# lightec-xyz/bls-verify-gadget

Measured on AMD Instinct MI355X. Metric: BLS-verify witness instances/sec (full pairing circuit), higher is better.
Workload: dtype u32 (381-bit Montgomery integers mod the BLS12-381 prime as 12 x 32-bit limbs in memory, products on 14 x 28-bit limbs with 64-bit columns; SHA-256 words)

## Files before the change

__graft_entry__.py:

```python
import importlib
import os
import subprocess
import sys

ROOT = os.path.dirname(os.path.abspath(__file__))
if ROOT not in sys.path:
    sys.path.insert(0, ROOT)


def build():
    pkg = importlib.import_module("bls-verify-gadget_amd")
    pkg.build(force=False)
    subprocess.check_call(["make", "-s", "-C", os.path.join(ROOT, "oracle")])
    subprocess.check_call(["make", "-s", "-C", os.path.join(ROOT, "tests", "hostsim")])
    subprocess.check_call(["make", "-s", "-C", os.path.join(ROOT, "tests", "vgroups")])
    subprocess.check_call(["make", "-s", "-j3", "-C", os.path.join(ROOT, "tests", "devfield")])
    subprocess.check_call(["make", "-s", "-j3", "-C", os.path.join(ROOT, "tests", "devcurve")])
    subprocess.check_call(["make", "-s", "-C", os.path.join(ROOT, "tests", "devteam")])
    subprocess.check_call(["make", "-s", "-C", os.path.join(ROOT, "tests", "devstream")])
    subprocess.check_call(["make", "-s", "-C", os.path.join(ROOT, "tests", "msg_input")])
    subprocess.check_call(["make", "-s", "-C", os.path.join(ROOT, "tests", "agg_inputs")])
    subprocess.check_call(["make", "-s", "-C", os.path.join(ROOT, "tests", "c_caller")])
    subprocess.check_call(["make", "-s", "-C", os.path.join(ROOT, "tests", "cpp_caller")])
    pkg.lib()
    for s in pkg.EXPORTED_SYMBOLS:
        getattr(pkg.lib(), s)


def smoke():
    import numpy as np
    import torch

    from tests import oracle_lib, synth

    pkg = importlib.import_module("bls-verify-gadget_amd")
    o = oracle_lib.load()
    n = 4
    pk, msg, sig, expect = synth.make_batch(o, n, seed=0x5EED)
    dev = torch.device("cuda:0")
    g = pkg.BlsSignatureVerifyGadget(n, 32, device=dev)
    res = g.verify(pkg.ParametersVar(), pkg.PublicKeyVar.new_witness(torch.from_numpy(pk.view(np.int64)).to(dev)),
                   torch.from_numpy(msg).to(dev), pkg.SignatureVar.new_witness(torch.from_numpy(sig.view(np.int64)).to(dev)))
    torch.cuda.synchronize()
    got = res.cpu().numpy().astype(bool)
    w = g.witness.cpu().numpy().view(np.uint64)
    for i in range(n):
        nw, _, r, ow = o.witness(pk[i], msg[i].tobytes(), sig[i])
# ... 10 lines not shown
```

bls-verify-gadget_amd/csrc/engine.hip:

```cpp
#include <cstdio>
#include <cstdlib>
#include <deque>
#include <map>
#include <vector>
#include "kcommon.hpp"
#include "agg_input.hpp"

using namespace blsw;

namespace {

inline int hip_ok(hipError_t e, const char* what) {
    if (e != hipSuccess) {
        fprintf(stderr, "[blsw] %s: %s\n", what, hipGetErrorString(e));
        return BLSW_ERR_HIP;
    }
    return BLSW_OK;
}

struct DeviceGuard {
    int prev = -1;
    bool switched = false;
    explicit DeviceGuard(int dev) {
        if (dev < 0) return;
// ... 85 lines not shown
    for (int k = 0; k < BLSW_MAX_BUFFERS; k++) {
        GroupBuf& b = e->buf[k];
        if (b.h_desc) hipHostFree(b.h_desc);
        if (b.d_desc) hipFree(b.d_desc);
        for (int i = 0; i < 2; i++)
            if (b.st[i]) hipStreamDestroy(b.st[i]);
        hipEvent_t single[] = {b.ev_start, b.ev_aux, b.ev_sha, b.ev_chains, b.ev_done, b.ev_side};
        for (hipEvent_t ev : single)
            if (ev) hipEventDestroy(ev);
        for (hipEvent_t ev : b.ev_cof)
            if (ev) hipEventDestroy(ev);
        hipEvent_t* arrays[] = {b.ev_in, b.ev_x, b.ev_step};
        for (hipEvent_t* arr : arrays) {
            if (!arr) continue;
            for (uint32_t s = 0; s < e->max_steps; s++)
                if (arr[s]) hipEventDestroy(arr[s]);
            delete[] arr;
        }
    }
    if (e->sha) hipStreamDestroy(e->sha);
    if (e->expand) hipStreamDestroy(e->expand);
    if (e->place) hipStreamDestroy(e->place);
    if (e->lat) hipStreamDestroy(e->lat);
    if (e->ev_exp) {
        for (int i = 0; i < 2 * BLSW_MAX_TIMED; i++)
            if (e->ev_exp[i]) hipEventDestroy(e->ev_exp[i]);
        delete[] e->ev_exp;
    }
    for (int i = 0; i < BLSW_MAX_CONSUMED; i++)
        if (e->consumed_ev[i]) hipEventDestroy(e->consumed_ev[i]);
    delete e;
}

static void launch_place(blsw_engine* e, hipStream_t st, const Fp* staging, const Fp* pair, uint32_t split_row, uint64_t first, uint64_t* out, uint64_t out_stride) {
    const blsw_layout_t& R = e->LR;
    const uint32_t rows = R.n_witness - R.sha_bits;
    const unsigned chunks = (rows * 3 + 256 * BLSW_PLACE_ITERS - 1) / (256 * BLSW_PLACE_ITERS);
    dim3 grid2(8 * ((chunks + 7) / 8) * (unsigned)e->n);
    const MovedSegment mv = moved_segment(R, e->modes);
    hipLaunchKernelGGL(k_place_field, grid2, dim3(256), 0, st, staging, pair, first, R.off_expand, R.sha_bits, rows, split_row, out + (uint64_t)e->head * 6, out_stride,
                       (uint32_t)e->n, mv.lo, mv.len, mv.at);
}
static void launch_place_multi(blsw_engine* e, hipStream_t st, const Workspace& ws, const Fp* pair_tiles, uint64_t first_pair, const Fp* inst_tiles, uint64_t first_inst,
                               uint32_t inst_tile_w, const Fp* rows, uint64_t* out, uint64_t out_stride) {
    const blsw_layout_t& L = e->L;
    const blsw_layout_t& S = e->LS;
    const uint32_t K = L.n_pairs, n = (uint32_t)e->n;
    PlaceRuns pr = {};
    pr.n_runs = 6;
    const uint32_t src[7] = {S.off_msg, S.off_pk_alloc, S.off_pk_not_zero, S.off_map0, S.off_prep_h, S.off_prep_pk, ws.rows_p};
    const uint32_t dst[6] = {L.off_msg, L.off_pk_alloc, L.off_pk_not_zero, L.off_map0, L.off_prep_h, L.off_prep_pk};
    const uint32_t str[6] = {L.stride_msg, L.stride_pk_alloc, L.stride_pk_not_zero, L.stride_hash, L.stride_prep_h, L.stride_prep_pk};
    for (int r = 0; r < 7; r++) pr.src_row[r] = src[r];
    for (int r = 0; r < 6; r++) pr.dst_off[r] = dst[r], pr.dst_stride[r] = str[r];
    auto blocks = [](uint32_t rows_, uint32_t n_y) {
        const unsigned chunks = (rows_ * 3 + 256 * BLSW_PLACE_ITERS - 1) / (256 * BLSW_PLACE_ITERS);
        return dim3(8 * ((chunks + 7) / 8) * n_y);
    };
    hipLaunchKernelGGL(k_place_runs, blocks(ws.rows_p, n * K), dim3(256), 0, st, pair_tiles, first_pair, ws.rows_p, pr, out, out_stride, n * K, K, 64u);
    PlaceRuns pi = {};
    pi.n_runs = 2;
    pi.src_row[0] = S.off_sig_alloc;
    pi.src_row[1] = S.off_prep_sig;
    pi.src_row[2] = ws.rows_i;
    pi.dst_off[0] = L.off_sig_alloc;
    pi.dst_off[1] = L.off_prep_sig;
    hipLaunchKernelGGL(k_place_runs, blocks(ws.rows_i, n), dim3(256), 0, st, inst_tiles, first_inst, ws.rows_i, pi, out, out_stride, n, 1u, inst_tile_w);
    const unsigned chunks = (ws.pair_rows * 3 + 256 * BLSW_PLACE_ITERS - 1) / (256 * BLSW_PLACE_ITERS);
    hipLaunchKernelGGL(k_place_rows, dim3(chunks, n), dim3(256), 0, st, rows, ws.pair_rows, L.off_miller, out, out_stride);
}
static void launch_canonical(blsw_engine* e, hipStream_t st, uint64_t* out, uint64_t out_stride) {
    const blsw_layout_t& R = e->LR;
    const uint32_t K = R.n_pairs, rows = R.n_witness - K * R.sha_bits;
    hipLaunchKernelGGL(k_canonical_rows, dim3((rows + 255) / 256, (unsigned)e->n), dim3(256), 0, st, out + (uint64_t)e->head * 6, out_stride, R.off_expand, R.sha_bits, rows, K,
// ... 29 lines not shown
        e->consumed_live[c] = false;
    }
}
static void materialise(blsw_engine* e, int k, uint32_t s) {
    GroupBuf& b = e->buf[k];
    const StepDesc& d = b.h_desc[s];
    const Workspace& ws = b.ws;
    const uint32_t Kc = e->L.n_pairs;
    const CompactForm cf = compact_form(e->n, ws, Kc);
    hipStreamWaitEvent(e->expand, b.ev_sha, 0);
    if (d.compact) {
        wait_released(e, e->expand, d.compact);
        hipMemcpyAsync(d.compact, ws.bits + (uint64_t)s * (e->n * Kc / 64) * bits_tile_words(ws.sha_words), cf.bits_bytes, hipMemcpyDeviceToDevice, e->expand);
    }
    if (d.out) {
        wait_released(e, e->expand, d.out);
        const bool timed = e->n_timed < BLSW_MAX_TIMED;
        if (timed) hipEventRecord(e->ev_exp[2 * e->n_timed], e->expand);
        const uint32_t K = e->L.n_pairs;
        ExpandArgs xa = {ws.bits, ws.sha_words, (uint64_t)s * e->n * K, e->L.sha_bits, e->L.off_expand, d.out, d.out_stride, K, K > 1 ? e->L.stride_hash : 0u, 0, (int)e->opt.output_form};
        if (b.lat_group && e->opt.consumer_mode) hipStreamWaitEvent(e->expand, b.ev_cof[2 * BLSW_COFV_NSEG + 3], 0);
        engine_expand(e, e->expand, xa, (unsigned)(e->n * K));
        if (timed) {
            hipEventRecord(e->ev_exp[2 * e->n_timed + 1], e->expand);
            e->n_timed++;
        }
        if (e->head) launch_keys_broadcast(d.ks_table, e->head, d.out, d.out_stride, e->n, 0, e->expand);
    }
    hipEventRecord(b.ev_x[s], e->expand);
    hipStreamWaitEvent(e->place, b.ev_chains, 0);
    hipStreamWaitEvent(e->place, b.ev_x[s], 0);
    if (d.compact) {
        char* dst = reinterpret_cast<char*>(d.compact);
        hipMemcpyAsync(dst + cf.off_staging, ws.staging + (uint64_t)s * (e->n * Kc / 64) * ws.rows_p * 64, cf.staging_bytes, hipMemcpyDeviceToDevice, e->place);
        if (cf.inst_bytes) {
            const uint64_t lane0 = (uint64_t)s * e->n;
            const Fp* src = ws.staging_inst + (lane0 >> 6) * (uint64_t)ws.rows_i * 64 + (lane0 & 63);
            if (cf.inst_tile_w == 64)
                hipMemcpyAsync(dst + cf.off_inst, src, cf.inst_bytes, hipMemcpyDeviceToDevice, e->place);
            else
                hipMemcpy2DAsync(dst + cf.off_inst, e->n * sizeof(Fp), src, 64 * sizeof(Fp), e->n * sizeof(Fp), ws.rows_i, hipMemcpyDeviceToDevice, e->place);
        }
        if (cf.pair_bytes) hipMemcpyAsync(dst + cf.off_pair, ws.pair + (uint64_t)s * e->n * ws.pair_rows, cf.pair_bytes, hipMemcpyDeviceToDevice, e->place);
    }
    if (d.out && e->staged) {
        if (e->L.n_pairs > 1)
            launch_place_multi(e, e->place, ws, ws.staging, (uint64_t)s * e->n * e->L.n_pairs, ws.staging_inst, (uint64_t)s * e->n, 64u,
                               ws.pair + (uint64_t)s * e->n * ws.pair_rows, d.out, d.out_stride);
        else
            launch_place(e, e->place, ws.staging, ws.pair, ws.split_row, (uint64_t)s * e->n, d.out, d.out_stride);
    }
    if (d.out && e->opt.output_form) launch_canonical(e, e->place, d.out, d.out_stride);
    hipEventRecord(b.ev_step[s], e->place);
}
static int pump(blsw_engine* e) {
    while (!e->jobs.empty()) {
        const Job j = e->jobs.front();
        GroupBuf& b = e->buf[j.buf];
        const StepDesc& d = b.h_desc[j.s];
        const void* ptr = tracked_output(e, d);
        int slot = -1;
        if (ptr) {
            slot = consumed_slot(e, ptr);
            if (slot < 0) return BLSW_ERR_ARG;
            if (e->held[slot]) break;
        }
        materialise(e, j.buf, j.s);
        if (slot >= 0) {
            e->held[slot] = true;
            e->refs[slot]--;
        }
        e->jobs.pop_front();
        e->materialised++;
        if (--b.jobs_left == 0) hipEventRecord(b.ev_done, e->place);
    }
    return hip_ok(hipGetLastError(), "materialise");
}

static bool group_trace_on() {
    static const bool on = getenv("BLSW_TRACE_GROUP") != nullptr;
    return on;
}
static void group_trace_mark(GroupTrace* t, int i, hipStream_t st) {
// ... 545 lines not shown
                                         void* d_compact, int32_t* d_result, uint32_t* d_count, void* stream_) {
    if (!e || !e->L.n_keys || e->head || !e->staged || e->n % 64 || !d_compact || !d_pks_xy || !d_bitmap || !d_sig_xy || (!d_msg && e->msg_len)) return BLSW_ERR_ARG;
    StepDesc d = {nullptr, d_sig_xy, d_msg, nullptr, 0, d_result, d_pks_xy, d_bitmap, d_count, d_compact};
    return engine_submit(e, d, stream_);
}
int blsw_engine_submit_aggregate_keyset_compact(blsw_engine_t* e, const blsw_keyset_t* ks, const uint8_t* d_bitmap, const uint64_t* d_sig_xy, const uint8_t* d_msg,
                                                void* d_compact, int32_t* d_result, uint32_t* d_count, void* stream_) {
    if (!keyset_fits(e, ks) || !e->staged || e->n % 64 || !d_compact || !d_bitmap || !d_sig_xy || (!d_msg && e->msg_len)) return BLSW_ERR_ARG;
    StepDesc d = {nullptr, d_sig_xy, d_msg, nullptr, 0, d_result, nullptr, d_bitmap, d_count, d_compact, nullptr, nullptr,
                  reinterpret_cast<const uint64_t*>(ks->table), ks->proj};
    return engine_submit(e, d, stream_);
}
int blsw_engine_submit_multi_compact(blsw_engine_t* e, const uint64_t* d_pks_xy, const uint8_t* d_msgs, const uint64_t* d_sig_xy, void* d_compact, int32_t* d_result,
                                     void* stream_) {
    if (!e || e->L.n_pairs < 2 || !compact_shape_ok(e->n, e->L.n_pairs) || !d_compact || !d_pks_xy || !d_sig_xy || (!d_msgs && e->msg_len)) return BLSW_ERR_ARG;
    StepDesc d = {d_pks_xy, d_sig_xy, d_msgs, nullptr, 0, d_result, nullptr, nullptr, nullptr, d_compact, nullptr};
    return engine_submit(e, d, stream_);
}
static int expand_compact(blsw_engine_t* e, const blsw_keyset* ks, const void* d_compact, uint64_t* d_witness, uint64_t witness_stride, void* stream_) {
    if (!e || !e->staged || !compact_shape_ok(e->n, e->L.n_pairs) || !d_compact || !d_witness || witness_stride < e->L.n_witness) return BLSW_ERR_ARG;
    DeviceGuard guard(e->device);
    hipStream_t st = reinterpret_cast<hipStream_t>(stream_);
    const uint32_t K = e->L.n_pairs;
    const Workspace w = carve(nullptr, e->n * K, e->LR, true, e->modes, e->n);
    if (ks) launch_keys_broadcast(reinterpret_cast<const uint64_t*>(ks->table), e->head, d_witness, witness_stride, e->n, 0, st);
    const CompactForm cf = compact_form(e->n, w, K);
    const char* src = reinterpret_cast<const char*>(d_compact);
    ExpandArgs xa = {reinterpret_cast<const uint32_t*>(src), w.sha_words, 0, e->L.sha_bits, e->L.off_expand, d_witness, witness_stride, K, K > 1 ? e->L.stride_hash : 0u, 0, (int)e->opt.output_form};
    engine_expand(e, st, xa, (unsigned)(e->n * K));
    if (K > 1)
        launch_place_multi(e, st, w, reinterpret_cast<const Fp*>(src + cf.off_staging), 0, reinterpret_cast<const Fp*>(src + cf.off_inst), 0, cf.inst_tile_w,
                           reinterpret_cast<const Fp*>(src + cf.off_pair), d_witness, witness_stride);
    else
        launch_place(e, st, reinterpret_cast<const Fp*>(src + cf.off_staging), reinterpret_cast<const Fp*>(src + cf.off_pair), w.split_row, 0, d_witness, witness_stride);
    if (e->opt.output_form) launch_canonical(e, st, d_witness, witness_stride);
    return hip_ok(hipGetLastError(), "expand compact");
}
int blsw_engine_expand_compact(blsw_engine_t* e, const void* d_compact, uint64_t* d_witness, uint64_t witness_stride, void* stream_) {
    if (!e || e->head) return BLSW_ERR_ARG;
    return expand_compact(e, nullptr, d_compact, d_witness, witness_stride, stream_);
}
int blsw_engine_expand_compact_keyset(blsw_engine_t* e, const blsw_keyset_t* ks, const void* d_compact, uint64_t* d_witness, uint64_t witness_stride, void* stream_) {
    if (!keyset_fits(e, ks)) return BLSW_ERR_ARG;
    return expand_compact(e, ks, d_compact, d_witness, witness_stride, stream_);
}

static uint64_t keyset_offsets(uint32_t n_keys, uint64_t* off_proj) {
    *off_proj = align_up((uint64_t)n_keys * SEG_PK_ALLOC * sizeof(Fp), 256);
    return *off_proj + align_up(3ull * n_keys * sizeof(Fp), 256);
}
int blsw_keyset_bytes(uint32_t n_keys, uint64_t* bytes) {
    if (!bytes || n_keys == 0 || n_keys > 65535) return BLSW_ERR_ARG;
    uint64_t off_proj;
    *bytes = keyset_offsets(n_keys, &off_proj);
    return BLSW_OK;
}
int blsw_keyset_create(blsw_keyset_t** out, const uint64_t* d_pks_xy, uint32_t n_keys, uint32_t output_form, int32_t device, void* d_buffer, uint64_t buffer_bytes,
                       void* stream_) {
    uint64_t need = 0, off_proj = 0;
    if (!out || !d_pks_xy || !d_buffer || output_form > 1 || blsw_keyset_bytes(n_keys, &need) || buffer_bytes < need || (reinterpret_cast<uintptr_t>(d_buffer) & 255))
        return BLSW_ERR_ARG;
    *out = nullptr;
    int ndev = 0;
    if (hipGetDeviceCount(&ndev) != hipSuccess || ndev == 0) return BLSW_ERR_NO_DEVICE;
    int dev = device;
    if (dev < 0 && hipGetDevice(&dev) != hipSuccess) return BLSW_ERR_NO_DEVICE;
    if (dev >= ndev) return BLSW_ERR_ARG;
// ... 504 lines not shown
```

bls-verify-gadget_amd/csrc/gadgets.hpp:

```cpp
#pragma once
#include "fp.hpp"

namespace blsw {

#if defined(__HIPCC__)
typedef uint32_t blsw_u32x4 __attribute__((ext_vector_type(4)));
typedef __attribute__((address_space(1))) blsw_u32x4 blsw_global_u32x4;
#endif
struct Emitter {
    uint32_t* base;
    uint32_t pos;
    uint64_t stride = 12;
    BLSW_HD void store_at(uint32_t at, const Fp& v) const {
#if defined(__HIP_DEVICE_COMPILE__)
        blsw_global_u32x4* d = (blsw_global_u32x4*)(base + (size_t)at * stride);
        d[0] = blsw_u32x4{v.l[0], v.l[1], v.l[2], v.l[3]};
        d[1] = blsw_u32x4{v.l[4], v.l[5], v.l[6], v.l[7]};
        d[2] = blsw_u32x4{v.l[8], v.l[9], v.l[10], v.l[11]};
#else
        uint32_t* d = base + (size_t)at * stride;
        for (int i = 0; i < 12; i++) d[i] = v.l[i];
#endif
    }
    BLSW_HD void put(const Fp& v) {
        if (base == nullptr) {
            pos++;
            return;
        }
#ifdef BLSW_QUAD_DEV
        if (quad_role() == 0)
#endif
            store_at(pos, v);
        pos++;
    }
#ifdef BLSW_QUAD_DEV
    BLSW_HD void put_split(const Fp& mine, uint32_t n) {
        const uint32_t role = quad_role();
        if (base != nullptr && role < n) store_at(pos + role, mine);
        pos += n;
    }
#endif
    BLSW_HD void put_bool(bool b) {
        Fp one = fp_one();
        Fp v;
#pragma unroll
        for (int i = 0; i < 12; i++) v.l[i] = b ? one.l[i] : 0u;
        put(v);
    }
};

BLSW_HD Fp fp_mul_w(Emitter& e, const Fp& a, const Fp& b) {
    Fp r = fp_mul(a, b);
    e.put(r);
    return r;
// ... 165 lines not shown
```

bls-verify-gadget_amd/csrc/k_stream.hip:

```cpp
#include "kcommon.hpp"

namespace blsw {

typedef uint32_t u32x4 __attribute__((ext_vector_type(4)));
template <int NT>
__device__ __forceinline__ void expand_store(uint4* dst, const uint4& v) {
    if (NT == 2) {
        u32x4 vv = {v.x, v.y, v.z, v.w};
        asm volatile("global_store_dwordx4 %0, %1, off sc1\n\ts_nop 1" ::"v"(dst), "v"(vv) : "memory");
    } else if (NT == 3) {
        u32x4 vv = {v.x, v.y, v.z, v.w};
        asm volatile("global_store_dwordx4 %0, %1, off sc0 sc1\n\ts_nop 1" ::"v"(dst), "v"(vv) : "memory");
    } else if (NT == 1) {
        __builtin_nontemporal_store(v.x, &dst->x);
        __builtin_nontemporal_store(v.y, &dst->y);
        __builtin_nontemporal_store(v.z, &dst->z);
        __builtin_nontemporal_store(v.w, &dst->w);
    } else {
        *dst = v;
    }
}
__device__ __forceinline__ uint4 expand_column(uint32_t c, int canonical) {
    if (canonical) return make_uint4(c == 0 ? 1u : 0u, 0u, 0u, 0u);
    constexpr uint32_t R1[12] = BLSW_R1_LIMBS;
// ... 180 lines not shown
    for (int k = 0; k < ITERS; k++) {
        const uint32_t m = (uint32_t)__builtin_amdgcn_sbfe(window(k), idx, 1);
        const u32x4 v = {rc.x & m, rc.y & m, rc.z & m, rc.w & m};
        if (e0 + (THREADS / 3) * k < a.sha_bits) expand_store_s(sbase + (uint64_t)k * (THREADS * 16), voff, v);
    }
}
void launch_expand(uint32_t variant, uint32_t store, unsigned lds, hipStream_t st, ExpandArgs a, unsigned n_y) {
    a.prio = (variant >> 8) & 1;
    const uint32_t n_pieces = a.sha_bits * 3;
    auto grid = [&](uint32_t per_wg) { return dim3((n_pieces + per_wg - 1) / per_wg + 1, n_y); };
    switch (variant & 0xff) {
        case 1: hipLaunchKernelGGL((k_sha_expand_chunk<256, 0>), grid(256), dim3(256), lds, st, a); break;
        case 6: hipLaunchKernelGGL((k_sha_expand_chunk<512, 0>), grid(512), dim3(512), lds, st, a); break;
        case 7: hipLaunchKernelGGL((k_sha_expand_chunk<1024, 0>), grid(1024), dim3(1024), lds, st, a); break;
        case 8: hipLaunchKernelGGL(k_sha_expand_s<8>, grid(384 * 8), dim3(384), lds, st, a); break;
        case 9: hipLaunchKernelGGL(k_sha_expand_s<4>, grid(384 * 4), dim3(384), lds, st, a); break;
        case 10: hipLaunchKernelGGL(k_sha_expand_l<8>, grid(384 * 8), dim3(384), lds, st, a); break;
        case 11: hipLaunchKernelGGL(k_sha_expand_l<16>, grid(384 * 16), dim3(384), lds, st, a); break;
        case 12: hipLaunchKernelGGL(k_sha_expand_l<32>, grid(384 * 32), dim3(384), lds, st, a); break;
        case 13: hipLaunchKernelGGL((k_sha_expand_resident<384, 8, 16, 0>), dim3(BLSW_EXPAND_RESIDENT_WGS), dim3(384), lds, st, a, grid(384 * 8).x, n_y); break;
        case 2: hipLaunchKernelGGL((k_sha_expand<768, 8, 256, 0>), grid(768 * 8), dim3(768), lds, st, a); break;
        case 3: hipLaunchKernelGGL((k_sha_expand<768, 4, 256, 0>), grid(768 * 4), dim3(768), lds, st, a); break;
        case 4: hipLaunchKernelGGL((k_sha_expand<768, 16, 256, 0>), grid(768 * 16), dim3(768), lds, st, a); break;
        case 5: hipLaunchKernelGGL((k_sha_expand<384, 16, 256, 0>), grid(384 * 16), dim3(384), lds, st, a); break;
        default:
            switch (store) {
                case 1: hipLaunchKernelGGL((k_sha_expand<384, 8, 16, 1>), grid(384 * 8), dim3(384), lds, st, a); break;
                case 2: hipLaunchKernelGGL((k_sha_expand<384, 8, 16, 2>), grid(384 * 8), dim3(384), lds, st, a); break;
                case 3: hipLaunchKernelGGL((k_sha_expand<384, 8, 16, 3>), grid(384 * 8), dim3(384), lds, st, a); break;
                default: hipLaunchKernelGGL((k_sha_expand<384, 8, 16, 0>), grid(384 * 8), dim3(384), lds, st, a); break;
            }
    }
}
__global__ __launch_bounds__(256) void k_place_field(const Fp* __restrict__ staging, const Fp* __restrict__ pair, uint64_t first, uint32_t off_expand,
                                                     uint32_t sha_bits, uint32_t staging_rows, uint32_t split_row, uint64_t* __restrict__ d_witness,
                                                     uint64_t stride, uint32_t n_inst, uint32_t moved_lo, uint32_t moved_len, uint32_t moved_at) {
    const uint32_t L = blockIdx.x, s_in_xcd = L >> 3;
    const uint32_t chunk = (L & 7) + 8 * (s_in_xcd / n_inst);
    const uint64_t inst = s_in_xcd % n_inst;
    const uint32_t nchunks = staging_rows * 3;
    if (chunk * (256u * BLSW_PLACE_ITERS) >= nchunks) return;
    const uint64_t lane = first + inst;
    const uint4* src = reinterpret_cast<const uint4*>(staging + (lane >> 6) * (uint64_t)split_row * 64 + (lane & 63));
    const uint4* src2 = reinterpret_cast<const uint4*>(pair + lane * (uint64_t)(staging_rows - split_row));
    uint4* out = reinterpret_cast<uint4*>(d_witness + inst * stride * 6);
    uint32_t q0 = chunk * (256 * BLSW_PLACE_ITERS) + threadIdx.x;
#pragma unroll
    for (int k = 0; k < BLSW_PLACE_ITERS; k++) {
        uint32_t q = q0 + k * 256;
        if (q < nchunks) {
            uint32_t e = q / 3, c = q - e * 3;
            uint4 v = e < split_row ? src[(uint64_t)e * 64 * 3 + c] : src2[(uint64_t)(e - split_row) * 3 + c];
            uint32_t t = e;
            if (moved_len) t = e >= moved_at ? moved_lo + (e - moved_at) : (e >= moved_lo ? e + moved_len : e);
            uint32_t dst_e = (moved_len && e >= moved_at) ? t : (t < off_expand ? t : t + sha_bits);
            out[(uint64_t)dst_e * 3 + c] = v;
        }
    }
}

__global__ __launch_bounds__(256) void k_place_runs(const Fp* __restrict__ tiles, uint64_t first, uint32_t rows, PlaceRuns runs, uint64_t* __restrict__ d_witness,
                                                    uint64_t stride, uint32_t n_y, uint32_t K, uint32_t tile_w) {
    const uint32_t L = blockIdx.x, s_in_xcd = L >> 3;
    const uint32_t chunk = (L & 7) + 8 * (s_in_xcd / n_y);
    const uint32_t y = s_in_xcd % n_y;
    const uint32_t npieces = rows * 3;
    if (chunk * (256u * BLSW_PLACE_ITERS) >= npieces) return;
    const uint64_t lane = first + y;
    const uint32_t inst = y / K, j = y - inst * K;
    const uint4* src = reinterpret_cast<const uint4*>(tiles + (lane / tile_w) * (uint64_t)rows * tile_w + (lane % tile_w));
    uint4* out = reinterpret_cast<uint4*>(d_witness + (uint64_t)inst * stride * 6);
    const uint32_t q0 = chunk * (256 * BLSW_PLACE_ITERS) + threadIdx.x;
#pragma unroll
    for (int k = 0; k < BLSW_PLACE_ITERS; k++) {
        const uint32_t q = q0 + k * 256;
        if (q < npieces) {
            const uint32_t e = q / 3, c = q - e * 3;
            uint32_t r = 0;
#pragma unroll
            for (int t = 1; t < 6; t++) r += (t < (int)runs.n_runs && e >= runs.src_row[t]) ? 1u : 0u;
            const uint32_t dst_e = runs.dst_off[r] + j * runs.dst_stride[r] + (e - runs.src_row[r]);
            out[(uint64_t)dst_e * 3 + c] = src[(uint64_t)e * tile_w * 3 + c];
        }
    }
}
__global__ __launch_bounds__(256) void k_place_rows(const Fp* __restrict__ rows, uint32_t n_rows, uint32_t dst_off, uint64_t* __restrict__ d_witness, uint64_t stride) {
    const uint64_t inst = blockIdx.y;
    const uint4* src = reinterpret_cast<const uint4*>(rows + inst * n_rows);
    uint4* out = reinterpret_cast<uint4*>(d_witness + (inst * stride + dst_off) * 6);
    const uint32_t npieces = n_rows * 3;
// ... 83 lines not shown
```

bls-verify-gadget_amd/csrc/kcommon.hpp:

```cpp
#pragma once
#include <hip/hip_runtime.h>
#include <stdio.h>
#include <stdlib.h>
#include <string.h>
#define BLSW_ATTR_W2 __attribute__((amdgpu_waves_per_eu(2, 2)))
#if defined(BLSW_KVARIANT_QUAD)
#define BLSW_QUAD 1
#define BLSW_INLINE_CHAINS 1
#define BLSW_CHAIN_ATTR
#define BLSW_K(name) name##_q
#define BLSW_LPI 4u
#elif defined(BLSW_KVARIANT_INL)
#define BLSW_INLINE_CHAINS 1
#define BLSW_CHAIN_ATTR
#define BLSW_K(name) name##_inl
#define BLSW_LPI 1u
#else
#if defined(BLSW_CHAIN_W2) || defined(BLSW_CHAIN_FULL)
#define BLSW_INLINE_CHAINS 1
#endif
#ifdef BLSW_CHAIN_W2
#define BLSW_CHAIN_ATTR BLSW_ATTR_W2
#else
#define BLSW_CHAIN_ATTR
#endif
#define BLSW_K(name) name
#define BLSW_LPI 1u
#endif
#include "chains.hpp"
#include "cofactor_vf.hpp"
#include "prepare_vf.hpp"
#include "layout.h"

namespace blsw {

__device__ __forceinline__ uint64_t item_index() { return ((uint64_t)blockIdx.x * blockDim.x + threadIdx.x) / BLSW_LPI; }
__device__ __forceinline__ bool item_leader() { return BLSW_LPI == 1u || (threadIdx.x & (BLSW_LPI - 1u)) == 0u; }
inline unsigned item_grid(uint64_t items, unsigned lpi) { return (unsigned)((items * lpi + 63) / 64); }

struct Workspace {
    uint32_t* bits;
    Fp* u;
    Fp* q;
    Fp* h;
    Fp* pkaff;
    Fp* coeff_h;
    Fp* coeff_sig;
    uint64_t n_sig;
    Fp* keyproj;
    Fp* staging;
    Fp* staging_inst;
    uint32_t rows_p, rows_i;
    uint64_t staging_rows;
    Fp* pair;
    uint32_t split_row;
    uint32_t pair_rows;
    uint64_t sha_words;
    Fp* cofv;
    Fp* prepv_h;
    Fp* prepv_sig;
    uint64_t total_bytes;
};
#define BLSW_LATENCY_MAX_LANES 8192
inline uint64_t align_up(uint64_t x, uint64_t a) { return (x + a - 1) / a * a; }
BLSW_HD uint64_t bits_tile_words(uint64_t sha_words) { return sha_words * 64; }
struct Modes {
    bool pairing_team;
    bool g2_team;
};
constexpr Modes DEFAULT_MODES = {true, false};
inline blsw_layout_t staging_layout(const blsw_layout_t& L, const Modes& m) {
    blsw_layout_t S = L;
    uint32_t* f = &S.off_msg;
    const uint32_t* g = &L.off_msg;
    for (int k = 0; k < 15; k++) f[k] = g[k] > L.off_expand ? g[k] - L.sha_bits : g[k];
    if (L.off_prep_g1 > L.off_expand) S.off_prep_g1 = L.off_prep_g1 - L.sha_bits;
    if (m.g2_team) {
        const uint32_t lo = L.off_sig_alloc, len = L.off_pk_not_zero - L.off_sig_alloc;
        for (int k = 0; k < 15; k++)
            if (f[k] > lo) f[k] -= len;
        if (S.off_prep_g1 > lo) S.off_prep_g1 -= len;
        S.off_sig_alloc = L.n_witness - L.sha_bits - len;
    }
// ... 39 lines not shown
inline Workspace carve(void* base, uint64_t N, const blsw_layout_t& L, bool with_staging, const Modes& m, uint64_t n_sig = 0) {
    Workspace w;
    if (n_sig == 0) n_sig = N;
    w.sha_words = align_up((L.sha_bits + 31) / 32 + 1, BLSW_BITS_CHUNK_WORDS);
    uint64_t off = 0;
    auto take = [&](uint64_t bytes) {
        uint64_t o = off;
        off = align_up(off + bytes, 256);
        return reinterpret_cast<char*>(base) + o;
    };
    w.bits = reinterpret_cast<uint32_t*>(take(bits_tile_words(w.sha_words) * (align_up(N, 64) / 64) * 4));
    w.u = reinterpret_cast<Fp*>(take(4 * N * sizeof(Fp)));
    w.q = reinterpret_cast<Fp*>(take(12 * N * sizeof(Fp)));
    w.h = reinterpret_cast<Fp*>(take(6 * N * sizeof(Fp)));
    w.pkaff = reinterpret_cast<Fp*>(take(2 * N * sizeof(Fp)));
    w.coeff_h = reinterpret_cast<Fp*>(take(272ull * N * sizeof(Fp)));
    w.coeff_sig = reinterpret_cast<Fp*>(take(272ull * n_sig * sizeof(Fp)));
    w.n_sig = n_sig;
    w.keyproj = L.n_keys && !L.pk_mode ? reinterpret_cast<Fp*>(take(3ull * N * L.n_keys * sizeof(Fp))) : nullptr;
    const bool small = N <= BLSW_LATENCY_MAX_LANES;
    w.cofv = small ? reinterpret_cast<Fp*>(take((uint64_t)BLSW_COFV_ELEMS * N * sizeof(Fp))) : nullptr;
    w.prepv_h = small ? reinterpret_cast<Fp*>(take((uint64_t)BLSW_PREPV_ELEMS * N * sizeof(Fp))) : nullptr;
    w.prepv_sig = small ? reinterpret_cast<Fp*>(take((uint64_t)BLSW_PREPV_ELEMS * n_sig * sizeof(Fp))) : nullptr;
    w.staging_rows = L.n_witness - L.sha_bits;
    if (L.n_pairs > 1 && with_staging) {
        const MultiStaging ms = staging_layout_multi(L);
        w.rows_p = ms.rows_p;
        w.rows_i = ms.rows_i;
        w.split_row = ms.split;
        w.pair_rows = ms.pair_rows;
        w.staging = reinterpret_cast<Fp*>(take((uint64_t)w.rows_p * align_up(N, 64) * sizeof(Fp)));
        w.staging_inst = reinterpret_cast<Fp*>(take((uint64_t)w.rows_i * align_up(n_sig, 64) * sizeof(Fp)));
        w.pair = reinterpret_cast<Fp*>(take((uint64_t)w.pair_rows * n_sig * sizeof(Fp)));
        w.total_bytes = off;
        return w;
    }
    w.split_row = m.pairing_team ? staging_layout(L, m).off_miller : (uint32_t)w.staging_rows;
    w.pair_rows = (uint32_t)w.staging_rows - w.split_row;
    w.rows_p = w.rows_i = w.split_row;
    w.staging = with_staging ? reinterpret_cast<Fp*>(take((uint64_t)w.split_row * align_up(N, 64) * sizeof(Fp))) : nullptr;
    w.staging_inst = w.staging;
    w.pair = with_staging && w.pair_rows ? reinterpret_cast<Fp*>(take((uint64_t)w.pair_rows * N * sizeof(Fp))) : nullptr;
    w.total_bytes = off;
    return w;
}

struct StepDesc {
    const uint64_t* pk;
    const uint64_t* sig;
    const uint8_t* msg;
    uint64_t* out;
    uint64_t out_stride;
    int32_t* result;
    const uint64_t* keys;
    const uint8_t* bitmap;
    uint32_t* count;
    void* compact;
    const int32_t* status;
    uint64_t* inst;
    const uint64_t* ks_table;
    const Fp* ks_proj;
};
__device__ __forceinline__ int32_t step_result(const StepDesc& d, uint32_t i, bool res) {
    if (d.status && (d.status[2 * i] | d.status[2 * i + 1])) return 0;
    return res ? 1 : 0;
}
struct CompactForm {
    uint64_t bits_bytes, staging_bytes, inst_bytes, pair_bytes, off_staging, off_inst, off_pair, total;
    uint32_t inst_tile_w;
};
inline CompactForm compact_form(uint64_t n, const Workspace& w, uint32_t K = 1) {
    CompactForm c;
    c.bits_bytes = bits_tile_words(w.sha_words) * (n * K / 64) * 4;
    c.staging_bytes = (uint64_t)w.rows_p * n * K * sizeof(Fp);
// ... 99 lines not shown
__device__ __forceinline__ Fp2 ld_fp2(const Fp* p, uint64_t n) { return {ld_fp(p), ld_fp(p + n)}; }

struct LaneId {
    uint64_t I;
    uint32_t s, i, j, f;
};
__device__ __forceinline__ LaneId lane_id(const Group& g, uint64_t I) {
    LaneId r;
    r.I = I;
    const uint32_t nk = g.n * g.K;
    r.s = (uint32_t)(I / nk);
    r.f = (uint32_t)(I - (uint64_t)r.s * nk);
    r.i = g.K == 1 ? r.f : r.f / g.K;
    r.j = g.K == 1 ? 0u : r.f - r.i * g.K;
    return r;
}
__device__ __forceinline__ void put_instance(const Group& g, const LaneId& id, uint32_t k, const Fp& v) {
    uint64_t* base = g.desc[id.s].inst;
    if (!base) return;
    st_fp(reinterpret_cast<Fp*>(base) + ((uint64_t)id.i * g.L.n_instance_vars + k), g.canonical ? fp_to_canonical(v) : v);
}

__device__ __forceinline__ Emitter emitter(const Group& g, const LaneId& id, uint32_t off_full, uint32_t off_staging, bool per_pair) {
    Emitter e;
    if (g.ws.staging) {
        if (!per_pair && off_staging >= g.ws.split_row) {
            e.base = reinterpret_cast<uint32_t*>(g.ws.pair + id.I * g.ws.pair_rows);
            e.pos = off_staging - g.ws.split_row;
            e.stride = 12;
            return e;
        }
        Fp* tiles = per_pair ? g.ws.staging : g.ws.staging_inst;
        const uint32_t rows = per_pair ? g.ws.rows_p : g.ws.rows_i;
        e.base = reinterpret_cast<uint32_t*>(tiles + (id.I >> 6) * (uint64_t)rows * 64 + (id.I & 63));
        e.pos = off_staging;
        e.stride = 64 * 12;
        return e;
    }
    const StepDesc& d = g.desc[id.s];
    e.base = d.out ? reinterpret_cast<uint32_t*>(d.out + (uint64_t)id.i * d.out_stride * 6) : nullptr;
    e.pos = off_full;
    e.stride = 12;
    return e;
}
#define EMIT(g, id, field) emitter(g, id, (g).L.field, (g).LS.field, false)
#define EMITJ(g, id, field, stride) emitter(g, id, (g).L.field + (id).j * (g).L.stride, (g).LS.field + (id).j * (g).LS.stride, true)

__device__ __forceinline__ Proj<OpsFp2> ld_proj2(const Fp* p, uint64_t n) {
    Proj<OpsFp2> r;
    r.x = ld_fp2(p, n);
    r.y = ld_fp2(p + 2 * n, n);
    r.z = ld_fp2(p + 4 * n, n);
    return r;
}

struct CoeffStrided {
    Fp* p;
    uint64_t n;
    __device__ __forceinline__ void st(uint32_t idx, const Fp& v) const {
        if (item_leader()) st_fp(p + (uint64_t)idx * n, v);
    }
    __device__ __forceinline__ Fp ld(uint32_t idx) const { return ld_fp(p + (uint64_t)idx * n); }
};

struct ExpandArgs {
    const uint32_t* bits;
    uint64_t sha_words, first;
    uint32_t sha_bits, off_expand;
    uint64_t* d_witness;
// ... 16 lines not shown
#define BLSW_CHAIN_I(name, params) __global__ void name params; __global__ void name##_inl params;
#define BLSW_CHAIN_Q(name, params) __global__ void name params; __global__ void name##_q params;
#define BLSW_CHAIN_IQ(name, params) BLSW_CHAIN_I(name, params) __global__ void name##_q params;
BLSW_CHAIN_I(k_sha, (Group g, int want_bits, int write_u))
BLSW_CHAIN_I(k_g1, (Group g))
BLSW_CHAIN_I(k_agg_keys, (Group g, Fp* keyproj))
BLSW_CHAIN_I(k_agg_sum, (Group g, const Fp* keyproj))
BLSW_CHAIN_I(k_agg_sum_in, (Group g))
BLSW_CHAIN_I(k_agg_sum_ks, (Group g))
BLSW_CHAIN_I(k_cofactor, (Group g))
BLSW_CHAIN_I(k_cofactor_chunk, (Group g))
BLSW_CHAIN_I(k_cofactor_join, (Group g))
BLSW_CHAIN_IQ(k_g2_alloc, (Group g))
BLSW_CHAIN_IQ(k_map, (Group g))
BLSW_CHAIN_IQ(k_prepare, (Group g, int which))
BLSW_CHAIN_Q(k_prepv_chain, (Group g, int which))
__global__ void k_prepv_step_w(Group g, int which);
BLSW_CHAIN_Q(k_cofv_chain, (Group g, int s))
BLSW_CHAIN_Q(k_cofv_bwd, (Group g, int s))
BLSW_CHAIN_Q(k_cofv_acc, (Group g, int s))
BLSW_CHAIN_Q(k_cofv_az, (Group g))
__global__ void k_cofv_aff(Group g, uint32_t lo, uint32_t cnt);
__global__ void k_cofv_dbl_w(Group g);
__global__ void k_cofv_add_w(Group g);
__global__ void k_cofv_join(Group g);
__global__ void k_sha_values(Group g);
__global__ void k_msg_input(Group g);
__global__ void k_agg_instance(Group g, uint32_t n_elems, uint32_t s0);
__global__ void k_map_values(Group g);
__global__ void k_cofactor_values(Group g);
__global__ void k_place_field(const Fp* __restrict__ staging, const Fp* __restrict__ pair, uint64_t first, uint32_t off_expand, uint32_t sha_bits,
                              uint32_t staging_rows, uint32_t split_row, uint64_t* __restrict__ d_witness, uint64_t stride, uint32_t n_inst, uint32_t moved_lo,
                              uint32_t moved_len, uint32_t moved_at);
__global__ void k_canonical_rows(uint64_t* __restrict__ d_witness, uint64_t stride, uint32_t off_expand, uint32_t sha_bits, uint32_t rows, uint32_t K, uint32_t stride_hash);
__global__ void k_digest(const uint64_t* __restrict__ w, uint64_t stride, uint64_t n_words, uint64_t* __restrict__ digest);
__global__ void k_pairing(Group g);
__global__ void k_pairing_team(Group g);
__global__ void k_pairing_team_pv(Group g);
__global__ void k_g2_alloc_team(Group g);
__global__ void k_pairing_team_multi(Group gs, uint32_t K, uint64_t n_h);
__global__ void k_decode(const uint8_t* __restrict__ pk48, const uint8_t* __restrict__ sig96, uint64_t n, uint64_t* pk_xy, uint64_t* sig_xy, int32_t* status);
__global__ void k_h_to_affine(uint64_t n, Workspace ws, uint64_t* d_out);
__global__ void k_decode_points(uint32_t group, const uint8_t* __restrict__ in, uint64_t m, Fp* xy, int32_t* st);
__global__ void k_sum_points(uint32_t group, const Fp* __restrict__ xy, const int32_t* __restrict__ pst, uint32_t k, uint64_t n, uint8_t* out, int32_t* status);
__global__ void k_sign(uint64_t n, Workspace ws, const uint8_t* __restrict__ sk32, uint8_t* sig96, uint64_t* sig_xy, uint8_t* pk48, uint64_t* pk_xy, int32_t* status);
__global__ void k_bench_mad(uint32_t iters, uint32_t* out);
__global__ void k_bench_fill(uint4* __restrict__ dst, uint64_t n16);
__global__ void k_bench_fpmul(uint32_t iters, uint32_t* out);
__global__ void k_bench_fpmul32(uint32_t iters, uint32_t* out);
__global__ void k_bench_fpinv(uint32_t iters, uint32_t* out);
__global__ void k_bench_fp2mulw(uint32_t iters, uint32_t* out);
struct MillerParArgs {
    Fp* cprod;
    Fp* q;
    Fp* t;
    Fp* f1;
    Fp* ffinal;
    uint32_t K, B, C;
    uint64_t n_h;
    uint32_t spine_lane;
};
#define BLSW_MILLER_CHUNK_DEFAULT 12
inline MillerParArgs carve_miller_par(char* base, uint64_t n, uint32_t K, uint64_t* bytes = nullptr) {
    MillerParArgs a = {};
    a.K = K;
    a.B = BLSW_MILLER_CHUNK_DEFAULT;
// ... 164 lines not shown
```

Measured before the change: 129,300.

## Store staging tiles piece-major so lane stores coalesce across the wavefront

Result: slower. 121,400 (-6.1%).

```diff
diff --git a/__graft_entry__.py b/__graft_entry__.py
--- a/__graft_entry__.py
+++ b/__graft_entry__.py
@@ -13,6 +13,7 @@
     pkg.build(force=False)
     subprocess.check_call(["make", "-s", "-C", os.path.join(ROOT, "oracle")])
     subprocess.check_call(["make", "-s", "-C", os.path.join(ROOT, "tests", "hostsim")])
+    subprocess.check_call(["make", "-s", "-C", os.path.join(ROOT, "tests", "stagesim")])
     subprocess.check_call(["make", "-s", "-C", os.path.join(ROOT, "tests", "vgroups")])
     subprocess.check_call(["make", "-s", "-j3", "-C", os.path.join(ROOT, "tests", "devfield")])
     subprocess.check_call(["make", "-s", "-j3", "-C", os.path.join(ROOT, "tests", "devcurve")])
diff --git a/bls-verify-gadget_amd/csrc/engine.hip b/bls-verify-gadget_amd/csrc/engine.hip
--- a/bls-verify-gadget_amd/csrc/engine.hip
+++ b/bls-verify-gadget_amd/csrc/engine.hip
@@ -141,14 +141,15 @@
     delete e;
 }
 
-static void launch_place(blsw_engine* e, hipStream_t st, const Fp* staging, const Fp* pair, uint32_t split_row, uint64_t first, uint64_t* out, uint64_t out_stride) {
+static void launch_place(blsw_engine* e, hipStream_t st, const Fp* staging, bool piece_major, const Fp* pair, uint32_t split_row, uint64_t first, uint64_t* out,
+                         uint64_t out_stride) {
     const blsw_layout_t& R = e->LR;
     const uint32_t rows = R.n_witness - R.sha_bits;
     const unsigned chunks = (rows * 3 + 256 * BLSW_PLACE_ITERS - 1) / (256 * BLSW_PLACE_ITERS);
     dim3 grid2(8 * ((chunks + 7) / 8) * (unsigned)e->n);
     const MovedSegment mv = moved_segment(R, e->modes);
-    hipLaunchKernelGGL(k_place_field, grid2, dim3(256), 0, st, staging, pair, first, R.off_expand, R.sha_bits, rows, split_row, out + (uint64_t)e->head * 6, out_stride,
-                       (uint32_t)e->n, mv.lo, mv.len, mv.at);
+    hipLaunchKernelGGL(piece_major ? k_place_field_pm : k_place_field, grid2, dim3(256), 0, st, staging, pair, first, R.off_expand, R.sha_bits, rows, split_row,
+                       out + (uint64_t)e->head * 6, out_stride, (uint32_t)e->n, mv.lo, mv.len, mv.at);
 }
 static void launch_place_multi(blsw_engine* e, hipStream_t st, const Workspace& ws, const Fp* pair_tiles, uint64_t first_pair, const Fp* inst_tiles, uint64_t first_inst,
                                uint32_t inst_tile_w, const Fp* rows, uint64_t* out, uint64_t out_stride) {
@@ -244,7 +245,12 @@
     hipStreamWaitEvent(e->place, b.ev_x[s], 0);
     if (d.compact) {
         char* dst = reinterpret_cast<char*>(d.compact);
-        hipMemcpyAsync(dst + cf.off_staging, ws.staging + (uint64_t)s * (e->n * Kc / 64) * ws.rows_p * 64, cf.staging_bytes, hipMemcpyDeviceToDevice, e->place);
+        const Fp* tiles = ws.staging + (uint64_t)s * (e->n * Kc / 64) * ws.rows_p * 64;
+        if (ws.piece_major) {
+            const uint64_t n_rows = cf.staging_bytes / (64 * sizeof(Fp));
+            if (n_rows) hipLaunchKernelGGL(k_compact_tiles, dim3((unsigned)((n_rows + 3) / 4)), dim3(256), 0, e->place, tiles, n_rows, reinterpret_cast<Fp*>(dst + cf.off_staging));
+        } else
+            hipMemcpyAsync(dst + cf.off_staging, tiles, cf.staging_bytes, hipMemcpyDeviceToDevice, e->place);
         if (cf.inst_bytes) {
             const uint64_t lane0 = (uint64_t)s * e->n;
             const Fp* src = ws.staging_inst + (lane0 >> 6) * (uint64_t)ws.rows_i * 64 + (lane0 & 63);
@@ -260,7 +266,7 @@
             launch_place_multi(e, e->place, ws, ws.staging, (uint64_t)s * e->n * e->L.n_pairs, ws.staging_inst, (uint64_t)s * e->n, 64u,
                                ws.pair + (uint64_t)s * e->n * ws.pair_rows, d.out, d.out_stride);
         else
-            launch_place(e, e->place, ws.staging, ws.pair, ws.split_row, (uint64_t)s * e->n, d.out, d.out_stride);
+            launch_place(e, e->place, ws.staging, ws.piece_major, ws.pair, ws.split_row, (uint64_t)s * e->n, d.out, d.out_stride);
     }
     if (d.out && e->opt.output_form) launch_canonical(e, e->place, d.out, d.out_stride);
     hipEventRecord(b.ev_step[s], e->place);
@@ -872,7 +878,7 @@
         launch_place_multi(e, st, w, reinterpret_cast<const Fp*>(src + cf.off_staging), 0, reinterpret_cast<const Fp*>(src + cf.off_inst), 0, cf.inst_tile_w,
                            reinterpret_cast<const Fp*>(src + cf.off_pair), d_witness, witness_stride);
     else
-        launch_place(e, st, reinterpret_cast<const Fp*>(src + cf.off_staging), reinterpret_cast<const Fp*>(src + cf.off_pair), w.split_row, 0, d_witness, witness_stride);
+        launch_place(e, st, reinterpret_cast<const Fp*>(src + cf.off_staging), false, reinterpret_cast<const Fp*>(src + cf.off_pair), w.split_row, 0, d_witness, witness_stride);
     if (e->opt.output_form) launch_canonical(e, st, d_witness, witness_stride);
     return hip_ok(hipGetLastError(), "expand compact");
 }
diff --git a/bls-verify-gadget_amd/csrc/gadgets.hpp b/bls-verify-gadget_amd/csrc/gadgets.hpp
--- a/bls-verify-gadget_amd/csrc/gadgets.hpp
+++ b/bls-verify-gadget_amd/csrc/gadgets.hpp
@@ -7,19 +7,31 @@
 typedef uint32_t blsw_u32x4 __attribute__((ext_vector_type(4)));
 typedef __attribute__((address_space(1))) blsw_u32x4 blsw_global_u32x4;
 #endif
+#define BLSW_TILE_LANES 64u
+#define BLSW_TILE_ROW_U32 (BLSW_TILE_LANES * 12u)
+BLSW_HD constexpr uint32_t tile_piece_u32(uint32_t lane, uint32_t c) { return c * (BLSW_TILE_LANES * 4u) + lane * 4u; }
+
 struct Emitter {
     uint32_t* base;
     uint32_t pos;
-    uint64_t stride = 12;
+    uint32_t stride = 12;
+    bool tile = false;
     BLSW_HD void store_at(uint32_t at, const Fp& v) const {
+        constexpr uint32_t P1 = tile_piece_u32(0, 1), P2 = tile_piece_u32(0, 2);
+        uint32_t* p = base + (size_t)at * stride;
 #if defined(__HIP_DEVICE_COMPILE__)
-        blsw_global_u32x4* d = (blsw_global_u32x4*)(base + (size_t)at * stride);
-        d[0] = blsw_u32x4{v.l[0], v.l[1], v.l[2], v.l[3]};
-        d[1] = blsw_u32x4{v.l[4], v.l[5], v.l[6], v.l[7]};
-        d[2] = blsw_u32x4{v.l[8], v.l[9], v.l[10], v.l[11]};
+        blsw_global_u32x4* d = (blsw_global_u32x4*)p;
+        const blsw_u32x4 v0 = {v.l[0], v.l[1], v.l[2], v.l[3]}, v1 = {v.l[4], v.l[5], v.l[6], v.l[7]}, v2 = {v.l[8], v.l[9], v.l[10], v.l[11]};
+        d[0] = v0;
+        if (tile) {
+            d[P1 / 4] = v1;
+            d[P2 / 4] = v2;
+        } else {
+            d[1] = v1;
+            d[2] = v2;
+        }
 #else
-        uint32_t* d = base + (size_t)at * stride;
-        for (int i = 0; i < 12; i++) d[i] = v.l[i];
+        for (int i = 0; i < 4; i++) p[i] = v.l[i], p[(tile ? P1 : 4) + i] = v.l[4 + i], p[(tile ? P2 : 8) + i] = v.l[8 + i];
 #endif
     }
     BLSW_HD void put(const Fp& v) {
diff --git a/bls-verify-gadget_amd/csrc/k_stream.hip b/bls-verify-gadget_amd/csrc/k_stream.hip
--- a/bls-verify-gadget_amd/csrc/k_stream.hip
+++ b/bls-verify-gadget_amd/csrc/k_stream.hip
@@ -236,16 +236,19 @@
             }
     }
 }
-__global__ __launch_bounds__(256) void k_place_field(const Fp* __restrict__ staging, const Fp* __restrict__ pair, uint64_t first, uint32_t off_expand,
-                                                     uint32_t sha_bits, uint32_t staging_rows, uint32_t split_row, uint64_t* __restrict__ d_witness,
-                                                     uint64_t stride, uint32_t n_inst, uint32_t moved_lo, uint32_t moved_len, uint32_t moved_at) {
+template <bool PIECE_MAJOR>
+__device__ __forceinline__ void place_field(const Fp* __restrict__ staging, const Fp* __restrict__ pair, uint64_t first, uint32_t off_expand, uint32_t sha_bits,
+                                            uint32_t staging_rows, uint32_t split_row, uint64_t* __restrict__ d_witness, uint64_t stride, uint32_t n_inst,
+                                            uint32_t moved_lo, uint32_t moved_len, uint32_t moved_at) {
     const uint32_t L = blockIdx.x, s_in_xcd = L >> 3;
     const uint32_t chunk = (L & 7) + 8 * (s_in_xcd / n_inst);
     const uint64_t inst = s_in_xcd % n_inst;
     const uint32_t nchunks = staging_rows * 3;
     if (chunk * (256u * BLSW_PLACE_ITERS) >= nchunks) return;
     const uint64_t lane = first + inst;
-    const uint4* src = reinterpret_cast<const uint4*>(staging + (lane >> 6) * (uint64_t)split_row * 64 + (lane & 63));
+    const uint32_t l = (uint32_t)(lane & 63);
+    const uint4* src = reinterpret_cast<const uint4*>(staging + (lane >> 6) * (uint64_t)split_row * 64) + (PIECE_MAJOR ? tile_piece_u32(l, 0) / 4u : l * 3u);
+    constexpr uint32_t cstep = PIECE_MAJOR ? (tile_piece_u32(0, 1) - tile_piece_u32(0, 0)) / 4u : 1u;
     const uint4* src2 = reinterpret_cast<const uint4*>(pair + lane * (uint64_t)(staging_rows - split_row));
     uint4* out = reinterpret_cast<uint4*>(d_witness + inst * stride * 6);
     uint32_t q0 = chunk * (256 * BLSW_PLACE_ITERS) + threadIdx.x;
@@ -254,12 +257,41 @@
         uint32_t q = q0 + k * 256;
         if (q < nchunks) {
             uint32_t e = q / 3, c = q - e * 3;
-            uint4 v = e < split_row ? src[(uint64_t)e * 64 * 3 + c] : src2[(uint64_t)(e - split_row) * 3 + c];
+            uint4 v = e < split_row ? src[(uint64_t)e * 64 * 3 + c * cstep] : src2[(uint64_t)(e - split_row) * 3 + c];
             uint32_t t = e;
             if (moved_len) t = e >= moved_at ? moved_lo + (e - moved_at) : (e >= moved_lo ? e + moved_len : e);
             uint32_t dst_e = (moved_len && e >= moved_at) ? t : (t < off_expand ? t : t + sha_bits);
             out[(uint64_t)dst_e * 3 + c] = v;
         }
+    }
+}
+__global__ __launch_bounds__(256) void k_place_field(const Fp* __restrict__ staging, const Fp* __restrict__ pair, uint64_t first, uint32_t off_expand,
+                                                     uint32_t sha_bits, uint32_t staging_rows, uint32_t split_row, uint64_t* __restrict__ d_witness,
+                                                     uint64_t stride, uint32_t n_inst, uint32_t moved_lo, uint32_t moved_len, uint32_t moved_at) {
+    place_field<false>(staging, pair, first, off_expand, sha_bits, staging_rows, split_row, d_witness, stride, n_inst, moved_lo, moved_len, moved_at);
+}
+__global__ __launch_bounds__(256) void k_place_field_pm(const Fp* __restrict__ staging, const Fp* __restrict__ pair, uint64_t first, uint32_t off_expand,
+                                                        uint32_t sha_bits, uint32_t staging_rows, uint32_t split_row, uint64_t* __restrict__ d_witness,
+                                                        uint64_t stride, uint32_t n_inst, uint32_t moved_lo, uint32_t moved_len, uint32_t moved_at) {
+    place_field<true>(staging, pair, first, off_expand, sha_bits, staging_rows, split_row, d_witness, stride, n_inst, moved_lo, moved_len, moved_at);
+}
+__global__ __launch_bounds__(256) void k_compact_tiles(const Fp* __restrict__ tiles, uint64_t n_rows, Fp* __restrict__ dst) {
+    __shared__ uint4 buf[4][192];
+    const uint32_t w = threadIdx.x >> 6, l = threadIdx.x & 63;
+    const uint64_t row = (uint64_t)blockIdx.x * 4 + w;
+    const bool live = row < n_rows;
+    const uint4* src = reinterpret_cast<const uint4*>(tiles) + row * 192;
+    uint4* out = reinterpret_cast<uint4*>(dst) + row * 192;
+    if (live) {
+#pragma unroll
+        for (uint32_t c = 0; c < 3; c++) buf[w][c * 64 + l] = src[c * 64 + l];
+    }
+    __syncthreads();
+    if (!live) return;
+#pragma unroll
+    for (uint32_t k = 0; k < 3; k++) {
+        const uint32_t j = k * 64 + l, lane = j / 3, c = j - lane * 3;
+        out[j] = buf[w][tile_piece_u32(lane, c) / 4u];
     }
 }
 
diff --git a/bls-verify-gadget_amd/csrc/kcommon.hpp b/bls-verify-gadget_amd/csrc/kcommon.hpp
--- a/bls-verify-gadget_amd/csrc/kcommon.hpp
+++ b/bls-verify-gadget_amd/csrc/kcommon.hpp
@@ -49,6 +49,7 @@
     uint64_t n_sig;
     Fp* keyproj;
     Fp* staging;
+    bool piece_major;
     Fp* staging_inst;
     uint32_t rows_p, rows_i;
     uint64_t staging_rows;
@@ -154,6 +155,7 @@
         w.staging = reinterpret_cast<Fp*>(take((uint64_t)w.rows_p * align_up(N, 64) * sizeof(Fp)));
         w.staging_inst = reinterpret_cast<Fp*>(take((uint64_t)w.rows_i * align_up(n_sig, 64) * sizeof(Fp)));
         w.pair = reinterpret_cast<Fp*>(take((uint64_t)w.pair_rows * n_sig * sizeof(Fp)));
+        w.piece_major = false;
         w.total_bytes = off;
         return w;
     }
@@ -162,6 +164,7 @@
     w.rows_p = w.rows_i = w.split_row;
     w.staging = with_staging ? reinterpret_cast<Fp*>(take((uint64_t)w.split_row * align_up(N, 64) * sizeof(Fp))) : nullptr;
     w.staging_inst = w.staging;
+    w.piece_major = with_staging;
     w.pair = with_staging && w.pair_rows ? reinterpret_cast<Fp*>(take((uint64_t)w.pair_rows * N * sizeof(Fp))) : nullptr;
     w.total_bytes = off;
     return w;
@@ -327,9 +330,11 @@
         }
         Fp* tiles = per_pair ? g.ws.staging : g.ws.staging_inst;
         const uint32_t rows = per_pair ? g.ws.rows_p : g.ws.rows_i;
-        e.base = reinterpret_cast<uint32_t*>(tiles + (id.I >> 6) * (uint64_t)rows * 64 + (id.I & 63));
+        const uint32_t l = (uint32_t)(id.I & 63);
+        e.base = reinterpret_cast<uint32_t*>(tiles + (id.I >> 6) * (uint64_t)rows * 64) + (g.ws.piece_major ? tile_piece_u32(l, 0) : l * 12u);
         e.pos = off_staging;
-        e.stride = 64 * 12;
+        e.stride = BLSW_TILE_ROW_U32;
+        e.tile = g.ws.piece_major;
         return e;
     }
     const StepDesc& d = g.desc[id.s];
@@ -412,6 +417,10 @@
 __global__ void k_place_field(const Fp* __restrict__ staging, const Fp* __restrict__ pair, uint64_t first, uint32_t off_expand, uint32_t sha_bits,
                               uint32_t staging_rows, uint32_t split_row, uint64_t* __restrict__ d_witness, uint64_t stride, uint32_t n_inst, uint32_t moved_lo,
                               uint32_t moved_len, uint32_t moved_at);
+__global__ void k_place_field_pm(const Fp* __restrict__ staging, const Fp* __restrict__ pair, uint64_t first, uint32_t off_expand, uint32_t sha_bits,
+                                 uint32_t staging_rows, uint32_t split_row, uint64_t* __restrict__ d_witness, uint64_t stride, uint32_t n_inst, uint32_t moved_lo,
+                                 uint32_t moved_len, uint32_t moved_at);
+__global__ void k_compact_tiles(const Fp* __restrict__ tiles, uint64_t n_rows, Fp* __restrict__ dst);
 __global__ void k_canonical_rows(uint64_t* __restrict__ d_witness, uint64_t stride, uint32_t off_expand, uint32_t sha_bits, uint32_t rows, uint32_t K, uint32_t stride_hash);
 __global__ void k_digest(const uint64_t* __restrict__ w, uint64_t stride, uint64_t n_words, uint64_t* __restrict__ digest);
 __global__ void k_pairing(Group g);
```
